# robjermy/CMVS-PMVS

Measured on AMD Instinct MI355X. Metric: refined patches/sec + NCC evals/sec, 50-view 4K synthetic, 1/2/4/8 GPU, higher is better.
Workload: dtype f32 (f64 optimizer)

## Files before the change

cmvs-pmvs_amd/csrc/pmvs_api.cpp:

```cpp
#include <hip/hip_runtime.h>

#include <algorithm>
#include <climits>
#include <cmath>
#include <cstdarg>
#include <cstdio>
#include <cstdlib>
#include <cstring>
#include <chrono>
#include <condition_variable>
#include <mutex>
#include <string>
#include <vector>

#include "../../include/pmvs_amd.h"
#include "pmvs_features.h"
#include "pmvs_fmt.h"
#include "pmvs_launch.h"

using namespace pmvsdev;

namespace {

thread_local std::string g_err = "";
// ... 763 lines not shown
  }
  pmvs_status st = check_candidates(sc, in, n);
  if (st) return st;
  HIPCHK(hipSetDevice(sc->device));
  if ((st = ensure(sc->cand, n)) || (st = ensure(sc->res, n))) return st;
  HIPCHK(hipMemcpyAsync(sc->cand.p, in, n * sizeof(pmvs_candidate), hipMemcpyHostToDevice, sc->stream));
  if ((st = pmvs_refine_batch_device(sc, sc->cand.p, n, sc->res.p))) return st;
  HIPCHK(hipMemcpyAsync(out, sc->res.p, n * sizeof(pmvs_refined), hipMemcpyDeviceToHost, sc->stream));
  return pmvs_scene_sync(sc, stats);
}

pmvs_status pmvs_selftest_math(int32_t device, int32_t op, const double* in, double* out, int32_t n) {
  if (!in || !out || n <= 0) return fail(PMVS_EINVAL, "null argument");
  HIPCHK(hipSetDevice(device));
  double *di = nullptr, *dout = nullptr;
  HIPCHK(hipMalloc((void**)&di, n * sizeof(double)));
  hipError_t e = hipMalloc((void**)&dout, n * sizeof(double));
  if (e == hipSuccess) e = hipMemcpy(di, in, n * sizeof(double), hipMemcpyHostToDevice);
  if (e == hipSuccess) e = launch_math_selftest(op, di, dout, n, nullptr);
  if (e == hipSuccess) e = hipMemcpy(out, dout, n * sizeof(double), hipMemcpyDeviceToHost);
  (void)hipFree(di);
  if (dout) (void)hipFree(dout);
  if (e != hipSuccess) return fail(PMVS_EDEVICE, "math selftest: %s", hipGetErrorString(e));
  return PMVS_OK;
}

pmvs_status pmvs_selftest_lls(int32_t device, const float* A, const float* b, const int32_t* offsets, int32_t nsys,
                              float* x) {
  if (!A || !b || !offsets || !x || nsys <= 0) return fail(PMVS_EINVAL, "null argument");
  for (int k = 0; k < nsys; ++k)
    if (offsets[k + 1] - offsets[k] < 5) return fail(PMVS_EINVAL, "system %d has fewer than 5 rows", k);
  HIPCHK(hipSetDevice(device));
  HIPCHK(lls_selftest(A, b, offsets, nsys, offsets[nsys], x));
  return PMVS_OK;
}

pmvs_status pmvs_selftest_bobyqa(int32_t device, int32_t mode, int32_t kind, const double* x0, int32_t n,
                                 int32_t maxeval, double* out, double* ms) {
  if (!x0 || !out || n <= 0) return fail(PMVS_EINVAL, "null argument");
  HIPCHK(hipSetDevice(device));
  double *dx = nullptr, *dout = nullptr;
  hipEvent_t e0 = nullptr, e1 = nullptr;
  HIPCHK(hipMalloc((void**)&dx, 3 * n * sizeof(double)));
  hipError_t e = hipMalloc((void**)&dout, 6 * n * sizeof(double));
  if (e == hipSuccess) e = hipEventCreate(&e0);
  if (e == hipSuccess) e = hipEventCreate(&e1);
  if (e == hipSuccess) e = hipMemcpy(dx, x0, 3 * n * sizeof(double), hipMemcpyHostToDevice);
  if (e == hipSuccess) e = hipEventRecord(e0, nullptr);
  if (e == hipSuccess) e = launch_bobyqa_selftest(mode, kind, dx, n, maxeval, dout, nullptr);
  if (e == hipSuccess) e = hipEventRecord(e1, nullptr);
  if (e == hipSuccess) e = hipMemcpy(out, dout, 6 * n * sizeof(double), hipMemcpyDeviceToHost);
  float t = 0;
  if (e == hipSuccess) e = hipEventElapsedTime(&t, e0, e1);
  if (ms) *ms = t;
  if (e0) (void)hipEventDestroy(e0);
  if (e1) (void)hipEventDestroy(e1);
  (void)hipFree(dx);
  if (dout) (void)hipFree(dout);
  if (e != hipSuccess) return fail(PMVS_EDEVICE, "bobyqa selftest: %s", hipGetErrorString(e));
  return PMVS_OK;
}

}

pmvs_status pmvs_patch_colors(pmvs_scene* sc, int32_t n, const float* coords4, const int32_t* nimg,
                              const int32_t* images_flat, int32_t* colors_out) {
// ... 957 lines not shown
```

cmvs-pmvs_amd/csrc/pmvs_filter.hip:

```cpp
#include <hip/hip_runtime.h>
#include <hipcub/hipcub.hpp>

#include <algorithm>
#include <chrono>
#include <cmath>
#include <cstdio>
#include <cstddef>
#include <cstdlib>
#include <cstring>
#include <functional>
#include <mutex>
#include <unordered_map>
#include <vector>

#include "pmvs_device.h"
#include "pmvs_launch.h"
#include "pmvs_layout.h"
#include "pmvs_queue.h"

namespace pmvsdev {

#ifndef PMVS_NB_CAP
#define PMVS_NB_CAP 1024
#endif
// ... 2647 lines not shown
  FCHK(memset_big(B.cellcnt, 0, (c.ncells + 1) * sizeof(int), c.st));
  if (e > 0) {
    hipLaunchKernelGGL(cell_hist_kernel, dim3(nblk(e)), dim3(256), 0, c.st, B.keys2, e, B.cellcnt);
    hipLaunchKernelGGL(items_kernel, dim3(nblk(e)), dim3(256), 0, c.st, B.keys2, e, items);
  }
  FCHK(cub_run(B.temp, [&](void* t, size_t& tb) {
    return hipcub::DeviceScan::ExclusiveSum(t, tb, B.cellcnt.p, csr_off, (int)(c.ncells + 1), c.st);
  }));
  return hipGetLastError();
}

__global__ void flag_order_kernel(const int* __restrict__ v, const int* __restrict__ order, int na, int* __restrict__ f) {
  const int i = blockIdx.x * blockDim.x + threadIdx.x;
  if (i < na) f[i] = v[order[i]] != 0;
}
__global__ void scatter_order_kernel(const int* __restrict__ f, const int* __restrict__ off, const int* __restrict__ order,
                                     int na, int* __restrict__ out) {
  const int i = blockIdx.x * blockDim.x + threadIdx.x;
  if (i < na && f[i]) out[off[i]] = order[i];
}

__global__ void pack_bits_kernel(const int* __restrict__ f, int n, unsigned* __restrict__ bits) {
  const int w = blockIdx.x * blockDim.x + threadIdx.x;
  if (w * 32 >= n) return;
  unsigned v = 0u;
  for (int b = 0; b < 32 && w * 32 + b < n; ++b) v |= (f[w * 32 + b] != 0 ? 1u : 0u) << b;
  bits[w] = v;
}
__global__ void unpack_bits_kernel(const unsigned* __restrict__ bits, int n, int* __restrict__ f) {
  const int k = blockIdx.x * blockDim.x + threadIdx.x;
  if (k < n) f[k] = (bits[k >> 5] >> (k & 31)) & 1u;
}

static int lab_jump() {
  static const int v = getenv("PMVS_LAB_JUMP") ? std::max(1, atoi(getenv("PMVS_LAB_JUMP"))) : 1;
  return v;
}
__global__ void lab_init_kernel(int* __restrict__ lab, int* __restrict__ active, int na) {
  const int i = blockIdx.x * blockDim.x + threadIdx.x;
  if (i < na) {
    lab[i] = i;
    active[i] = 1;
  }
}
__global__ void lab_relax_kernel(const int* __restrict__ eoff, const int* __restrict__ edges, int na, int* lab,
                                 int* active, int all, int* changed, int jump) {
  const int i = blockIdx.x * blockDim.x + threadIdx.x;
  if (i >= na) return;
  if (!all && !jump && active[i] == 0) return;
  const int l0 = lab[i], l1 = lab[l0];
  const bool jumped = l1 < l0 && atomicMin(&lab[i], l1) > l1;
  if (jumped) atomicOr(changed, 1);
  if (!all && !jumped && active[i] == 0) return;
  if (atomicExch(&active[i], 0) == 0 && !all && !jumped) return;
  const int li = atomicAdd(&lab[i], 0);
  bool any = false;
  for (int e = eoff[i]; e < eoff[i + 1]; ++e) {
    const int j = edges[e];
    if (li < lab[j] && atomicMin(&lab[j], li) > li) {
      atomicOr(&active[j], 1);
      any = true;
    }
  }
  if (any) atomicOr(changed, 1);
}
__global__ void lab_count_kernel(const int* __restrict__ lab, int na, int* __restrict__ csize) {
  const int i = blockIdx.x * blockDim.x + threadIdx.x;
  const int l = (i < na) ? lab[i] : -1;
  const int l0 = __shfl(l, 0, 64);
  const unsigned long long same = __ballot(i < na && l == l0);
  if (i < na && l != l0) atomicAdd(&csize[l], 1);
  if ((threadIdx.x & 63) == 0 && same) atomicAdd(&csize[l0], (int)__popcll(same));
}
__global__ void lab_flags_kernel(const int* __restrict__ lab, const int* __restrict__ csize, const int* __restrict__ order,
                                 int na, int threshold, int* __restrict__ flags) {
  const int i = blockIdx.x * blockDim.x + threadIdx.x;
  if (i < na && csize[lab[i]] < threshold) flags[order[i]] = 1;
}

static hipError_t collect(Ctx& c) {
  FilterBuffers& B = c.B;
  FCHK(hipMemsetAsync(B.counters, 0, 8 * sizeof(int), c.st));
  hipLaunchKernelGGL(first_cell_kernel, dim3(std::min(nblk((long long)c.n * kLG), 2048u)), dim3(256), 0, c.st, c.s, c.P, c.n,
                     B.preg, B.tgoff, B.keys,
                     B.counters);
  FCHK(cub_run(B.temp, [&](void* t, size_t& tb) {
    return hipcub::DeviceRadixSort::SortKeys(t, tb, B.keys.p, B.keys2.p, c.n, 32, 32 + cell_bits(c.ncells), c.st);
  }));
  FCHK(read_int(B.counters, &c.nalive, c.st));
  FCHK(hipMemsetAsync(B.rank, 0xff, c.n * sizeof(int), c.st));
  if (c.nalive > 0)
    hipLaunchKernelGGL(rank_kernel, dim3(nblk(c.nalive)), dim3(256), 0, c.st, B.keys2, c.nalive, B.order, B.rank);
  hipLaunchKernelGGL(hot_kernel, dim3(nblk(c.n)), dim3(256), 0, c.st, c.s, c.P, c.n, B.hot);
  return hipGetLastError();
}

static hipError_t set_dm_vgrids(Ctx& c, int additive) {
// ... 232 lines not shown
    }
    fprintf(stderr, "[filter] neighbours: max unique %d, overflowed %d of %d; first: %d %d %d\n", mx, ov, c.nalive,
            cnts[ord[0]], c.nalive > 1 ? cnts[ord[1]] : 0, c.nalive > 2 ? cnts[ord[2]] : 0);
  }
  FCHK(read_int(B.counters + 3, overflow, st));
  if (part) {
    long long ovf = 0;
    FCHK(merge_flags(*overflow, &ovf));
    *overflow = (int)ovf;
    if (inject && inj_where == 'g') return hipErrorOutOfMemory;
  }
  {
    int errs[2] = {0, 0};
    FCHK(hipMemcpy(errs, B.counters + 6, 2 * sizeof(int), hipMemcpyDeviceToHost));
    if (errs[0]) {
      fprintf(stderr, "[filter] neighbor kernel bounds violations: %d (first code %d)\n", errs[0], errs[1]);
      return hipErrorIllegalAddress;
    }
  }
  FCHK(apply_flags(c, &counts[2]));
  FCHK(set_dm_vgrids(c, 1));
  if (c.nalive) {
    const int na = c.nalive;
    hipLaunchKernelGGL(group_edges_kernel, dim3(nblk(na)), dim3(256), 0, st, s, c.dev(), 0, B.edge_off, B.cnt, B.edges);
    FCHK(hipMemsetAsync(B.cnt + na, 0, sizeof(int), st));
    FCHK(cub_run(B.temp, [&](void* t, size_t& tb) { return hipcub::DeviceScan::ExclusiveSum(t, tb, B.cnt.p, B.edge_off.p, na + 1, st); }));
    int ne = 0;
    FCHK(read_int(B.edge_off + na, &ne, st));
    if ((size_t)ne > B.edges.cap) FCHK(B.edges.alloc((size_t)ne * 2));
    hipLaunchKernelGGL(group_edges_kernel, dim3(nblk(na)), dim3(256), 0, st, s, c.dev(), 1, B.edge_off, B.cnt, B.edges);
    const int threshold = std::max(20, na / 10000);
    int* lab = B.need;
    int* csize = B.list;
    int* changed = B.counters + 5;
    int* active = B.list;
    hipLaunchKernelGGL(lab_init_kernel, dim3(nblk(na)), dim3(256), 0, st, lab, active, na);
    int sweep = 0;
    for (int it = 0;; ++it) {
      const bool verify = (it % 9) == 8;
      FCHK(hipMemsetAsync(changed, 0, sizeof(int), st));
      for (int r = 0; r < (verify ? 1 : 8); ++r) {
        if (ne)
          hipLaunchKernelGGL(lab_relax_kernel, dim3(nblk(na)), dim3(256), 0, st, B.edge_off, B.edges, na, lab, active,
                             verify ? 1 : 0, changed, (sweep++ % lab_jump()) == 0 ? 1 : 0);
      }
      int ch = 0;
      FCHK(read_int(changed, &ch, st));
      if (verify && !ch) break;
      if (!verify && !ch) it = 9 * (it / 9) + 7;
      if (it > 9 * (na + 1)) return hipErrorIllegalState;
    }
    FCHK(hipMemsetAsync(csize, 0, na * sizeof(int), st));
    hipLaunchKernelGGL(lab_count_kernel, dim3(nblk(na)), dim3(256), 0, st, lab, na, csize);
    FCHK(hipMemsetAsync(B.flags, 0, n * sizeof(int), st));
    hipLaunchKernelGGL(lab_flags_kernel, dim3(nblk(na)), dim3(256), 0, st, lab, csize, B.order, na, threshold, B.flags);
    hipLaunchKernelGGL(flag_rank_kernel, dim3(nblk(na)), dim3(256), 0, st, dP, B.order, na);
    hipLaunchKernelGGL(clear_fixed_kernel, dim3(nblk(n)), dim3(256), 0, st, dP, n, B.flags);
    FCHK(apply_flags(c, &counts[3]));
  }
  dbg(st, "groups");
  FCHK(set_dm_vgrids(c, 1));
  FCHK(build_lists(c, 0));
  FCHK(collect(c));
  hipLaunchKernelGGL(keep_kernel, dim3(nblk(n)), dim3(256), 0, st, n, B.preg, B.rank, keep_dev);
  int lovf = 0;
  FCHK(read_int(B.counters + 8, &lovf, st));
  if (lovf) return hipErrorNotSupported;
  return hipGetLastError();
}

static void nb_prof_dump(const char* what) {
#if defined(NB_PROFILE)
  unsigned long long h[3][8];
  if (hipDeviceSynchronize() != hipSuccess || hipMemcpyFromSymbol(h, HIP_SYMBOL(g_nb_prof), sizeof(h)) != hipSuccess) return;
  fprintf(stderr, "{\"nb_prof\": \"%s\"", what);
  for (int k = 0; k < 3; ++k) {
    fprintf(stderr, ", \"k%d\": [", k);
    for (int i = 0; i < 8; ++i) fprintf(stderr, "%s%llu", i ? ", " : "", h[k][i]);
    fprintf(stderr, "]");
  }
  fprintf(stderr, "}\n");
  std::memset(h, 0, sizeof(h));
  (void)hipMemcpyToSymbol(HIP_SYMBOL(g_nb_prof), h, sizeof(h));
#else
// ... 1064 lines not shown
__global__ __launch_bounds__(64) void lls_selftest_kernel(const float* __restrict__ A, const float* __restrict__ b,
                                                          const int* __restrict__ off, int nsys, double* __restrict__ scratch,
                                                          float* __restrict__ x) {
  __shared__ NbLds L;
  const int sys = blockIdx.x;
  if (sys >= nsys) return;
  const int o = off[sys], n = off[sys + 1] - off[sys];
  double* M = scratch + (size_t)o * 6;
  double* r = M + (size_t)n * 5;
  for (int i = threadIdx.x; i < n; i += 64) {
    for (int j = 0; j < 5; ++j) M[(size_t)i * 5 + j] = (double)A[(size_t)(o + i) * 5 + j];
    r[i] = (double)b[o + i];
  }
  __threadfence_block();
  __syncthreads();
  lls5_wave(L, M, r, n);
  if (threadIdx.x < 5) x[(size_t)sys * 5 + threadIdx.x] = L.x[threadIdx.x];
}

hipError_t lls_selftest(const float* A, const float* b, const int* off, int nsys, int total, float* x) {
  DevBuf<float> dA, db, dx;
  DevBuf<int> doff;
  DevBuf<double> scr;
  FCHK(dA.alloc((size_t)total * 5)); FCHK(db.alloc((size_t)total)); FCHK(dx.alloc((size_t)nsys * 5));
  FCHK(doff.alloc((size_t)nsys + 1)); FCHK(scr.alloc((size_t)total * 6));
  FCHK(hipMemcpy(dA, A, (size_t)total * 5 * sizeof(float), hipMemcpyHostToDevice));
  FCHK(hipMemcpy(db, b, (size_t)total * sizeof(float), hipMemcpyHostToDevice));
  FCHK(hipMemcpy(doff, off, (size_t)(nsys + 1) * sizeof(int), hipMemcpyHostToDevice));
  hipLaunchKernelGGL(lls_selftest_kernel, dim3(nsys), dim3(64), 0, nullptr, dA.p, db.p, doff.p, nsys, scr.p, dx.p);
  FCHK(hipGetLastError());
  return hipMemcpy(x, dx, (size_t)nsys * 5 * sizeof(float), hipMemcpyDeviceToHost);
}

__global__ __launch_bounds__(64) void compact_kernel(const pmvs_patch* __restrict__ src, int n, const int* __restrict__ keep,
                                                     const int* __restrict__ pos, pmvs_patch* __restrict__ dst) {
  const int k = blockIdx.x;
  if (k >= n || !keep[k]) return;
  const unsigned* a = reinterpret_cast<const unsigned*>(&src[k]);
  unsigned* b = reinterpret_cast<unsigned*>(&dst[pos[k]]);
  for (int w = threadIdx.x; w < (int)(sizeof(pmvs_patch) / 4); w += 64) b[w] = a[w];
}

__global__ void fill_int_kernel(int* __restrict__ a, int n, int v) {
  const int k = blockIdx.x * blockDim.x + threadIdx.x;
  if (k < n) a[k] = v;
}

hipError_t compact_model(FilterBuffers& B, const pmvs_patch* src, int n, const int* keep, const CompactDst& dst_for,
                         int* nkept, hipStream_t st) {
  *nkept = 0;
  if (n <= 0) return hipSuccess;
  FCHK(B.reserve(n, B.cap_cells, 0, B.cap_grid));
  FCHK(hipMemcpyAsync(B.cnt, keep, n * sizeof(int), hipMemcpyDeviceToDevice, st));
  FCHK(hipMemsetAsync(B.cnt + n, 0, sizeof(int), st));
  FCHK(cub_run(B.temp, [&](void* t, size_t& tb) { return hipcub::DeviceScan::ExclusiveSum(t, tb, B.cnt.p, B.off.p, n + 1, st); }));
  FCHK(read_int(B.off + n, nkept, st));
  pmvs_patch* dst = nullptr;
  FCHK(dst_for(*nkept, &dst));
  if (*nkept > 0) hipLaunchKernelGGL(compact_kernel, dim3(n), dim3(64), 0, st, src, n, keep, B.off, dst);
  return hipGetLastError();
}

hipError_t fill_int(int* a, int n, int v, hipStream_t st) {
  if (n > 0) hipLaunchKernelGGL(fill_int_kernel, dim3(nblk(n)), dim3(256), 0, st, a, n, v);
  return hipGetLastError();
}
// ... 149 lines not shown
```

cmvs-pmvs_amd/csrc/pmvs_launch.h:

```cpp
#pragma once
#include <hip/hip_runtime.h>
#include "pmvs_device.h"
#include "pmvs_devbuf.h"
#include "pmvs_refine_layouts.h"
#include <functional>
#include <memory>
#include <utility>
#include <vector>

namespace pmvsdev {

inline hipError_t memset_big(void* p, int value, size_t bytes, hipStream_t st) {
  constexpr size_t kPiece = size_t(1) << 30;
  char* c = static_cast<char*>(p);
  for (size_t off = 0; off < bytes; off += kPiece) {
    const hipError_t e = hipMemsetAsync(c + off, value, bytes - off < kPiece ? bytes - off : kPiece, st);
    if (e != hipSuccess) return e;
  }
  return hipSuccess;
}
struct PinnedBuf {
  void* p = nullptr;
  size_t cap = 0;
  PinnedBuf() = default;
// ... 70 lines not shown
hipError_t export_order(const DScene& s, const pmvs_patch* P, int n, int max_gwidth, int* sorted, int* cnt_i, int* cnt_v,
                        hipStream_t st);

struct TextArrays {
  const float* fields = nullptr;
  const int* colors = nullptr;
  const long long *image_off = nullptr, *vimage_off = nullptr;
  const int *image_ids = nullptr, *vimage_ids = nullptr;
};
hipError_t text_offsets(int kind, const TextArrays& in, int n, long long header_bytes, long long* d_off, hipStream_t st);
hipError_t text_write(int kind, const TextArrays& in, int n, const long long* d_off, char* d_out, hipStream_t st);
hipError_t launch_format_selftest(int precision, const float* d_in, int n, char* d_out, int* d_len, hipStream_t st);

struct DepthMapArrays {
  int* patch = nullptr;
  float *depth = nullptr, *normal = nullptr, *ncc = nullptr;
};
hipError_t depth_map_pass(const DScene& s, const pmvs_patch* P, int n, const int* src, const long long* d_off,
                          long long cells, const DepthMapArrays& out, hipStream_t st);

struct alignas(64) PHot {
  float coord[4];
  float normal[4];
  float dscale, ncc, unit0, pad[5];
};
struct FilterBuffers {
  PinnedBuf pin;
  DevBuf<Reg> preg, vreg, safe;
  DevBuf<unsigned long long> keys, keys2, dpkey;
  DevBuf<long long> tgoff;
  DevBuf<int> cnt, off, cellcnt, pg_off, pg_items, vp_off, vp_items, order, rank, flags, need, list, counters, edge_off,
      edges;
  DevBuf<PHot> hot;
  DevBuf<double> scratch;
  DevBuf<char> temp;
  DevBuf<unsigned> rbits;
  DevBuf<float4> coordc;
  DevBuf<unsigned long long> vrows, used;
  DevBuf<float4> normalc;
  DevBuf<int> refpos;
  DevBuf<char> xr;
  DevBuf<float> qf;
  DevBuf<double> qrows;
  DevBuf<int4> qjobs;
  DevBuf<unsigned long long> qctr;
  DevBuf<unsigned long long> qkeys, qkeys2;
  DevBuf<int> qcrows, qoff;
  size_t cap_qrows = 0;
  DevBuf<int> ovf_items;
  DevBuf<double> scratch_big;
  int cap_n = 0, cap_grid = 0;
  long long cap_cells = 0;
  size_t cap_e = 0;
  hipError_t reserve(int n, long long ncells, int tnum, int grid);
  hipError_t ensure_entries(size_t e, int vis);
  void release() { *this = FilterBuffers(); }
};

hipError_t launch_filter_refimage(const DScene& s, pmvs_patch* P, const int* list, int m, int grid, hipStream_t stream,
                                  int* refpos = nullptr, int rank = 0, int world = 1);
hipError_t launch_apply_refpos(const DScene& s, pmvs_patch* P, const int* list, int m, const int* allpos, int world,
                               hipStream_t stream);

constexpr int kMaxWave = 65536;
struct CommitWork;
struct CommitWorkDelete {
// ... 54 lines not shown
  ExchangeDevFn exchange_dev;
};
hipError_t filter_pass(const DScene& s, FilterBuffers& B, pmvs_patch* dP, int n, long long ncells, const long long* h_tgoff,
                       int grid, hipStream_t st, int counts[4], int* overflow, int* keep_dev, const Shard* sh = nullptr,
                       bool* handled = nullptr);
hipError_t expand_pass(const DScene& s, FilterBuffers& B, ExpandBuffers& X, pmvs_patch*& dP, size_t& dP_cap, int n0,
                       const int* d_alive, int cap, long long ncells, const long long* h_tgoff, int wave, int cthr,
                       int flags, int grid, hipStream_t st, const RefineFn& refine, const Shard& sh, long long stats[8],
                       int* n_out, int min_cands = 0);
using CompactDst = std::function<hipError_t(int, pmvs_patch**)>;
hipError_t compact_model(FilterBuffers& B, const pmvs_patch* src, int n, const int* keep, const CompactDst& dst_for,
                         int* nkept, hipStream_t st);
hipError_t fill_int(int* a, int n, int v, hipStream_t st);
void d2h_stage_release(hipStream_t st);

struct ClusterMaps {
  const unsigned char* shared_t;
  const int* ids;
  const int* id2idx;
  int maxid;
};
struct ClusterBuffers {
  DevBuf<BRec> send, recv;
  DevBuf<pmvs_patch> ins;
  DevBuf<int> flags, pos, cnts;
  DevBuf<char> temp;
};
hipError_t drop_foreign(FilterBuffers& B, const pmvs_patch* src, int n, const CompactDst& dst_for, int* n_out,
                        hipStream_t st);
hipError_t cluster_exchange(const DScene& s, ClusterBuffers& CB, const ClusterMaps& cm, const pmvs_patch* src, int n,
                            pmvs_patch*& dst, size_t& dst_cap, int* n_out, const Shard& sh, hipStream_t st,
                            long long xstats[3], bool& agreed);
hipError_t lls_selftest(const float* A, const float* b, const int* off, int nsys, int total, float* x);

struct SeedInput {
  const pmvs_point* points;
  const int* npts;
  const int* vis_off;
  const int* vis;
  int sequence;
  float angle0;
  std::vector<const uint8_t*> mask_level;
  int batch, per_cell;
  int lookahead;
  int spec_near;
};
struct SeedOutput {
  std::vector<pmvs_patch> seeds;
  long long stats[8];
  double gen_ms = 0, refine_ms = 0, wall_ms = 0;
};
hipError_t seed_pass(const DScene& s, const std::vector<DView>& hv, const SeedInput& in, hipStream_t st,
                     const RefineFn& refine, SeedOutput& out);
}
```

cmvs-pmvs_amd/pmvs_amd.py:

```python
from __future__ import annotations

import ctypes as C
import os
from dataclasses import dataclass, field
from typing import List, Optional, Sequence

import numpy as np

HERE = os.path.dirname(os.path.abspath(__file__))
LIB_PATH = os.environ.get("PMVS_AMD_LIB", os.path.join(HERE, "libpmvs_amd.so"))

MAX_IMAGES = 128
MAX_TAU = 16

ACCEPTED, FAIL_PRE, FAIL_POST, FAIL_OVERFLOW = 0, 1, 2, 3
FIX_FOREIGN = 2

CANDIDATE_DTYPE = np.dtype(
    [("coord", "<f4", 4), ("normal", "<f4", 4), ("dscale", "<f4"), ("num_images", "<i4"),
     ("images", "<i4", MAX_IMAGES)], align=True)
REFINED_DTYPE = np.dtype(
    [("status", "<i4"), ("refine_code", "<i4"), ("evals", "<i4"), ("num_images", "<i4"),
     ("coord", "<f4", 4), ("normal", "<f4", 4), ("ncc", "<f4"), ("dscale", "<f4"), ("ascale", "<f4"),
     ("tmp", "<f4"), ("timages", "<i4"), ("reserved", "<i4"), ("images", "<i4", MAX_IMAGES),
# ... 103 lines not shown
               [(k, C.c_float) for k in ("threshold", "set_edge", "max_angle", "quad")] + \
               [(k, C.c_int32) for k in ("num_timages", "num_oimages", "num_bindexes")] + \
               [(k, C.POINTER(C.c_int32)) for k in ("timages", "oimages", "bindexes", "visdata2_offsets",
                                                      "visdata2")]


class SynthParams(C.Structure):
    _fields_ = [("num_views", C.c_int32), ("num_targets", C.c_int32), ("width", C.c_int32),
                ("height", C.c_int32), ("supersample", C.c_int32), ("level", C.c_int32),
                ("seed", C.c_uint64), ("ring_radius", C.c_double), ("height_offset", C.c_double),
                ("focal_scale", C.c_double), ("arc_step_deg", C.c_double), ("gain_sigma", C.c_double),
                ("bias_sigma", C.c_double), ("noise_sigma", C.c_double), ("lowtex", C.c_double),
                ("occluder_radius", C.c_double), ("render_first", C.c_int32), ("render_count", C.c_int32)]


HARD = dict(gain_sigma=0.15, bias_sigma=0.04, noise_sigma=0.08, lowtex=0.5, occluder_radius=0.3)


EXPORTS = ["pmvs_last_error", "pmvs_device_count", "pmvs_scene_create", "pmvs_scene_destroy",
           "pmvs_set_thresholds", "pmvs_scene_get_level", "pmvs_grab_tex", "pmvs_incc_eval",
           "pmvs_refine_batch", "pmvs_refine_batch_device", "pmvs_scene_sync", "pmvs_synth_ring",
           "pmvs_synth_candidates", "pmvs_selftest_math", "pmvs_selftest_bobyqa", "pmvs_camera_load",
           "pmvs_ppm_load", "pmvs_options_load", "pmvs_options_free", "pmvs_write_patches", "pmvs_write_pset",
           "pmvs_write_ply", "pmvs_patch_colors", "pmvs_filter_run",
           "pmvs_expand_run", "pmvs_expand_fetch", "pmvs_run_loop", "pmvs_loop_fetch", "pmvs_loop_hash",
           "pmvs_loop_export_sizes", "pmvs_loop_export", "pmvs_export_patches_sizes", "pmvs_export_patches",
           "pmvs_depth_map_layout", "pmvs_loop_depth_maps", "pmvs_depth_maps_patches", "pmvs_write_pfm",
           "pmvs_loop_text", "pmvs_text_patches", "pmvs_selftest_format",
           "pmvs_scene_set_shard", "pmvs_scene_set_shard_rccl", "pmvs_scene_set_cluster",
           "pmvs_scene_set_cluster_rccl", "pmvs_rccl_unique_id",
           "pmvs_rccl_create", "pmvs_rccl_destroy", "pmvs_rccl_allgather", "pmvs_rccl_allgather_device",
           "pmvs_tcp_create", "pmvs_tcp_allgather", "pmvs_tcp_destroy", "pmvs_thread_exchange_create",
           "pmvs_thread_exchange_ctx", "pmvs_thread_allgather", "pmvs_thread_exchange_destroy", "pmvs_detect_features",
           "pmvs_seed_run", "pmvs_seed_fetch", "pmvs_selftest_lls", "pmvs_image_load", "pmvs_pnm_mask_load", "pmvs_set_edge"]

ALLGATHER_FN = C.CFUNCTYPE(C.c_int, C.c_void_p, C.c_void_p, C.c_int64, C.c_void_p)

_lib = None


def load_library(path: str = LIB_PATH) -> C.CDLL:
    global _lib
    if _lib is not None:
        return _lib
    if not os.path.exists(path):
        raise RuntimeError(f"{path} not built: run `make -C cmvs-pmvs_amd` (no CPU fallback exists)")
    lib = C.CDLL(path)
    lib.pmvs_last_error.restype = C.c_char_p
    lib.pmvs_device_count.restype = C.c_int32
    lib.pmvs_scene_create.argtypes = [C.POINTER(SceneDesc), C.c_int32, C.POINTER(C.c_void_p)]
    lib.pmvs_scene_destroy.argtypes = [C.c_void_p]
    lib.pmvs_scene_destroy.restype = None
    lib.pmvs_set_thresholds.argtypes = [C.c_void_p, C.c_float, C.c_float, C.c_int32]
    lib.pmvs_scene_get_level.argtypes = [C.c_void_p, C.c_int32, C.c_int32, C.c_void_p,
                                         C.POINTER(C.c_int32), C.POINTER(C.c_int32)]
    lib.pmvs_grab_tex.argtypes = [C.c_void_p, C.c_void_p, C.c_int32, C.c_void_p, C.c_void_p]
    lib.pmvs_detect_features.argtypes = [C.c_void_p, C.c_int32, C.c_int32, C.c_void_p, C.c_int32,
                                         C.POINTER(C.c_int32)]
    lib.pmvs_seed_run.argtypes = [C.c_void_p, C.c_void_p, C.c_void_p, C.c_int32, C.c_void_p, C.c_int32,
                                  C.POINTER(C.c_int32), C.POINTER(SeedStats)]
    lib.pmvs_seed_fetch.argtypes = [C.c_void_p, C.c_void_p, C.c_int32]
    lib.pmvs_incc_eval.argtypes = [C.c_void_p, C.c_void_p, C.c_int32, C.c_void_p, C.POINTER(Stats)]
    lib.pmvs_refine_batch.argtypes = [C.c_void_p, C.c_void_p, C.c_int32, C.c_void_p, C.POINTER(Stats)]
    lib.pmvs_refine_batch_device.argtypes = [C.c_void_p, C.c_void_p, C.c_int32, C.c_void_p]
    lib.pmvs_scene_sync.argtypes = [C.c_void_p, C.POINTER(Stats)]
    lib.pmvs_synth_ring.argtypes = [C.POINTER(SynthParams), C.c_void_p, C.c_void_p, C.c_int32]
    lib.pmvs_synth_candidates.argtypes = [C.POINTER(SynthParams), C.c_void_p, C.c_int32, C.c_uint64,
                                          C.c_float, C.c_float, C.c_void_p]
    lib.pmvs_selftest_bobyqa.argtypes = [C.c_int32, C.c_int32, C.c_int32, C.c_void_p, C.c_int32, C.c_int32,
                                         C.c_void_p, C.POINTER(C.c_double)]
    lib.pmvs_selftest_lls.argtypes = [C.c_int32, C.c_void_p, C.c_void_p, C.c_void_p, C.c_int32, C.c_void_p]
    lib.pmvs_selftest_math.argtypes = [C.c_int32, C.c_int32, C.c_void_p, C.c_void_p, C.c_int32]
    lib.pmvs_camera_load.argtypes = [C.c_char_p, C.c_void_p]
    lib.pmvs_image_load.argtypes = [C.c_char_p, C.POINTER(C.c_int32), C.POINTER(C.c_int32), C.c_void_p]
    lib.pmvs_pnm_mask_load.argtypes = [C.c_char_p, C.POINTER(C.c_int32), C.POINTER(C.c_int32), C.c_void_p]
    lib.pmvs_set_edge.argtypes = [C.c_void_p, C.c_int32, C.c_int32, C.c_float, C.c_void_p]
    lib.pmvs_ppm_load.argtypes = [C.c_char_p, C.POINTER(C.c_int32), C.POINTER(C.c_int32), C.c_void_p]
    lib.pmvs_options_load.argtypes = [C.c_char_p, C.c_char_p, C.POINTER(C.POINTER(Options))]
    lib.pmvs_options_free.argtypes = [C.POINTER(Options)]
    lib.pmvs_options_free.restype = None
    lib.pmvs_write_patches.argtypes = [C.c_char_p, C.c_int32] + [C.c_void_p] * 5
    lib.pmvs_write_pset.argtypes = [C.c_char_p, C.c_int32, C.c_void_p]
    lib.pmvs_write_ply.argtypes = [C.c_char_p, C.c_int32, C.c_void_p, C.c_void_p]
    lib.pmvs_patch_colors.argtypes = [C.c_void_p, C.c_int32] + [C.c_void_p] * 4
    lib.pmvs_filter_run.argtypes = [C.c_void_p, C.c_void_p, C.c_int32, C.c_void_p, C.POINTER(FilterStats)]
    lib.pmvs_expand_run.argtypes = [C.c_void_p, C.c_void_p, C.c_void_p, C.c_int32, C.c_int32, C.c_int32, C.c_int32, C.c_int32,
                                    C.c_void_p, C.c_void_p, C.c_int32, C.POINTER(C.c_int32), C.POINTER(ExpandStats)]
    lib.pmvs_expand_fetch.argtypes = [C.c_void_p, C.c_void_p, C.c_void_p, C.c_int32]
    lib.pmvs_run_loop.argtypes = [C.c_void_p, C.c_void_p, C.c_int32, C.c_float, C.c_int32, C.c_int32, C.c_int32, C.c_int32,
                                  C.c_int32, C.POINTER(C.c_int32), C.c_void_p]
    lib.pmvs_loop_fetch.argtypes = [C.c_void_p, C.c_void_p, C.c_int32]
    lib.pmvs_loop_hash.argtypes = [C.c_void_p, C.POINTER(C.c_uint64)]
    lib.pmvs_loop_export_sizes.argtypes = [C.c_void_p, C.POINTER(ExportSizes)]
    lib.pmvs_loop_export.argtypes = [C.c_void_p, C.c_int32, C.c_void_p, C.POINTER(ExportBuffers)]
    lib.pmvs_export_patches_sizes.argtypes = [C.c_void_p, C.c_void_p, C.c_int32, C.POINTER(ExportSizes)]
    lib.pmvs_export_patches.argtypes = [C.c_void_p, C.c_void_p, C.c_int32, C.c_int32, C.c_void_p,
                                        C.POINTER(ExportBuffers)]
    lib.pmvs_depth_map_layout.argtypes = [C.c_void_p, C.c_void_p, C.c_void_p]
    lib.pmvs_loop_depth_maps.argtypes = [C.c_void_p, C.c_int32, C.POINTER(DepthMapBuffers)]
    lib.pmvs_depth_maps_patches.argtypes = [C.c_void_p, C.c_void_p, C.c_int32, C.c_int32, C.POINTER(DepthMapBuffers)]
    lib.pmvs_write_pfm.argtypes = [C.c_char_p, C.c_int32, C.c_int32, C.c_void_p]
    lib.pmvs_loop_text.argtypes = [C.c_void_p, C.c_int32, C.c_int32, C.c_void_p, C.c_void_p, C.c_int64,
                                   C.POINTER(C.c_int64)]
    lib.pmvs_text_patches.argtypes = [C.c_void_p, C.c_void_p, C.c_int32, C.c_int32, C.c_int32, C.c_void_p, C.c_void_p,
# ... 434 lines not shown
        parts.append(r)
    npts = np.array([len(p) for p in parts], np.int32)
    flat = np.concatenate(parts) if parts and npts.sum() else np.zeros(1, POINT_DTYPE)
    return np.ascontiguousarray(flat), npts


def selftest_math(op: int, x: np.ndarray, device: int = 0) -> np.ndarray:
    x = np.ascontiguousarray(x, np.float64)
    out = np.zeros_like(x)
    _check(load_library().pmvs_selftest_math(device, op, _ptr(x), _ptr(out), len(x)))
    return out


def selftest_format(precision: int, x: np.ndarray, device: int = 0):
    x = np.ascontiguousarray(x, np.float32).reshape(-1)
    out = np.zeros((len(x), 24), np.uint8)
    ln = np.zeros(len(x), np.int32)
    if len(x):
        _check(load_library().pmvs_selftest_format(device, precision, _ptr(x), len(x), _ptr(out), _ptr(ln)))
    raw = out.tobytes()
    return [raw[24 * i:24 * i + int(k)] for i, k in enumerate(ln)]


def selftest_lls(systems, device: int = 0) -> np.ndarray:
    A = np.ascontiguousarray(np.concatenate([np.asarray(a, np.float32).reshape(-1, 5) for a, _ in systems]))
    b = np.ascontiguousarray(np.concatenate([np.asarray(v, np.float32).reshape(-1) for _, v in systems]))
    off = np.zeros(len(systems) + 1, np.int32)
    off[1:] = np.cumsum([len(v) for _, v in systems])
    x = np.zeros((len(systems), 5), np.float32)
    _check(load_library().pmvs_selftest_lls(device, _ptr(A), _ptr(b), _ptr(off), len(systems), _ptr(x)))
    return x


def selftest_bobyqa(kind: int, x0: np.ndarray, mode: int = 0, maxeval: int = 1000, device: int = 0):
    x0 = np.ascontiguousarray(x0, np.float64).reshape(-1, 3)
    out = np.zeros((len(x0), 6), np.float64)
    ms = C.c_double()
    _check(load_library().pmvs_selftest_bobyqa(device, mode, kind, _ptr(x0), len(x0), maxeval, _ptr(out), C.byref(ms)))
    return out, ms.value


def camera_load(path: str) -> np.ndarray:
    out = np.zeros(12, np.float32)
    _check(load_library().pmvs_camera_load(path.encode(), _ptr(out)))
    return out.reshape(3, 4)


def ppm_load(path: str) -> np.ndarray:
    lib = load_library()
    w, h = C.c_int32(), C.c_int32()
    _check(lib.pmvs_ppm_load(path.encode(), C.byref(w), C.byref(h), None))
    img = np.zeros((h.value, w.value, 3), np.uint8)
    _check(lib.pmvs_ppm_load(path.encode(), C.byref(w), C.byref(h), _ptr(img)))
    return img


def image_load(path: str) -> np.ndarray:
    lib = load_library()
    w, h = C.c_int32(), C.c_int32()
    _check(lib.pmvs_image_load(path.encode(), C.byref(w), C.byref(h), None))
    img = np.zeros((h.value, w.value, 3), np.uint8)
    _check(lib.pmvs_image_load(path.encode(), C.byref(w), C.byref(h), _ptr(img)))
    return img


def mask_load(path: str) -> np.ndarray:
# ... 227 lines not shown
```

include/pmvs_amd.h:

```cpp
#ifndef PMVS_AMD_H
#define PMVS_AMD_H

#include <stdint.h>

#ifdef __cplusplus
extern "C" {
#endif

#define PMVS_MAX_IMAGES 128
#define PMVS_MAX_TARGETS 256
#define PMVS_MAX_TAU 16
#define PMVS_MAX_LEVEL 4
#define PMVS_MAX_NEIGHBOURS 16384

typedef enum pmvs_status {
  PMVS_OK = 0,
  PMVS_EINVAL = 1,
  PMVS_EDEVICE = 2,
  PMVS_ENOMEM = 3,
  PMVS_EUNSUPPORTED = 4
} pmvs_status;

typedef enum pmvs_candidate_status {
  PMVS_ACCEPTED = 0,
// ... 101 lines not shown

pmvs_status pmvs_set_thresholds(pmvs_scene* scene, float ncc, float ncc_before, int32_t depth);

pmvs_status pmvs_scene_get_level(pmvs_scene* scene, int32_t view, int32_t level, uint8_t* out,
                                 int32_t* width, int32_t* height);

typedef struct pmvs_point {
  float x, y, response;
  int32_t type;
} pmvs_point;

pmvs_status pmvs_detect_features(pmvs_scene* scene, int32_t view, int32_t fcsize, pmvs_point* out, int32_t cap,
                                 int32_t* n_out);

pmvs_status pmvs_grab_tex(pmvs_scene* scene, const pmvs_tex_query* q, int32_t n, float* out_tex,
                          int32_t* out_valid);

pmvs_status pmvs_incc_eval(pmvs_scene* scene, const pmvs_eval_query* q, int32_t n, double* out_f,
                           pmvs_stats* stats);

pmvs_status pmvs_refine_batch(pmvs_scene* scene, const pmvs_candidate* in, int32_t n,
                              pmvs_refined* out, pmvs_stats* stats);

pmvs_status pmvs_refine_batch_device(pmvs_scene* scene, const pmvs_candidate* d_in, int32_t n,
                                     pmvs_refined* d_out);
pmvs_status pmvs_scene_sync(pmvs_scene* scene, pmvs_stats* stats);


pmvs_status pmvs_selftest_math(int32_t device, int32_t op, const double* in, double* out, int32_t n);

pmvs_status pmvs_selftest_lls(int32_t device, const float* A, const float* b, const int32_t* offsets, int32_t nsys,
                              float* x);

pmvs_status pmvs_selftest_bobyqa(int32_t device, int32_t mode, int32_t kind, const double* x0, int32_t n,
                                 int32_t maxeval, double* out, double* ms);

typedef struct pmvs_patch {
  float coord[4], normal[4];
  float ncc, dscale, ascale, tmp;
  int32_t timages, flag, fix, num_images, num_vimages, dflag;
  int16_t images[PMVS_MAX_IMAGES];
  int16_t grids[PMVS_MAX_IMAGES][2];
  int16_t vimages[PMVS_MAX_IMAGES];
  int16_t vgrids[PMVS_MAX_IMAGES][2];
} pmvs_patch;

#define PMVS_FIX_FOREIGN 2

typedef struct pmvs_filter_stats {
  int64_t input, removed_outside, removed_exact, removed_neighbor, removed_groups, kept;
  double kernel_ms;
} pmvs_filter_stats;

pmvs_status pmvs_filter_run(pmvs_scene* scene, pmvs_patch* patches, int32_t n, int32_t* keep,
                            pmvs_filter_stats* stats);

#define PMVS_EXPAND_AFTER_SEEDS 1
#define PMVS_EXPAND_MAX_WAVES(n) ((int32_t)((uint32_t)(n) << 8))
typedef struct pmvs_expand_stats {
  int64_t parents, candidates, fail_prep, fail_pre, fail_post, fail_commit, added, waves;
  double wall_ms;
  int64_t refined, evals, tex_valid;
  double refine_ms;
  int64_t refine_launches;
  int64_t tex_valid_small;
  double refine_ms_small;
// ... 160 lines not shown
```

Before: 963,300.

## Use frontier worklist label propagation for filter group component labeling

Replaces the fixed full-sweep label propagation in the patch-group filter with a hybrid fixpoint. It runs full relax sweeps while many vertices are active, and switches to a compacted frontier list processed by 16-lane groups once the active set is small. Host readbacks happen only once per batch of sweeps. This cuts wasted full-grid sweeps and host syncs on long-tail convergence, at the cost of more control logic, atomics on list counters, and a workspace buffer. It also adds a labels selftest API and optional tracing.

```diff
diff --git a/cmvs-pmvs_amd/csrc/pmvs_api.cpp b/cmvs-pmvs_amd/csrc/pmvs_api.cpp
--- a/cmvs-pmvs_amd/csrc/pmvs_api.cpp
+++ b/cmvs-pmvs_amd/csrc/pmvs_api.cpp
@@ -819,6 +819,17 @@
     if (offsets[k + 1] - offsets[k] < 5) return fail(PMVS_EINVAL, "system %d has fewer than 5 rows", k);
   HIPCHK(hipSetDevice(device));
   HIPCHK(lls_selftest(A, b, offsets, nsys, offsets[nsys], x));
+  return PMVS_OK;
+}
+
+pmvs_status pmvs_labels_selftest(const int32_t* eoff, const int32_t* edges, int32_t n, int32_t* lab_out) {
+  if (!eoff || !lab_out || n <= 0 || eoff[0] != 0) return fail(PMVS_EINVAL, "null argument or empty graph");
+  for (int i = 0; i < n; ++i)
+    if (eoff[i + 1] < eoff[i]) return fail(PMVS_EINVAL, "edge offsets decrease at vertex %d", i);
+  if (eoff[n] > 0 && !edges) return fail(PMVS_EINVAL, "null argument");
+  for (int e = 0; e < eoff[n]; ++e)
+    if (edges[e] < 0 || edges[e] >= n) return fail(PMVS_EINVAL, "edge %d leaves the graph", e);
+  HIPCHK(labels_selftest(eoff, edges, n, lab_out));
   return PMVS_OK;
 }
 
diff --git a/cmvs-pmvs_amd/csrc/pmvs_filter.hip b/cmvs-pmvs_amd/csrc/pmvs_filter.hip
--- a/cmvs-pmvs_amd/csrc/pmvs_filter.hip
+++ b/cmvs-pmvs_amd/csrc/pmvs_filter.hip
@@ -2703,10 +2703,6 @@
   if (k < n) f[k] = (bits[k >> 5] >> (k & 31)) & 1u;
 }
 
-static int lab_jump() {
-  static const int v = getenv("PMVS_LAB_JUMP") ? std::max(1, atoi(getenv("PMVS_LAB_JUMP"))) : 1;
-  return v;
-}
 __global__ void lab_init_kernel(int* __restrict__ lab, int* __restrict__ active, int na) {
   const int i = blockIdx.x * blockDim.x + threadIdx.x;
   if (i < na) {
@@ -2715,15 +2711,18 @@
   }
 }
 __global__ void lab_relax_kernel(const int* __restrict__ eoff, const int* __restrict__ edges, int na, int* lab,
-                                 int* active, int all, int* changed, int jump) {
+                                 int* active, int all, int* changed, int* nact) {
   const int i = blockIdx.x * blockDim.x + threadIdx.x;
   if (i >= na) return;
-  if (!all && !jump && active[i] == 0) return;
   const int l0 = lab[i], l1 = lab[l0];
   const bool jumped = l1 < l0 && atomicMin(&lab[i], l1) > l1;
   if (jumped) atomicOr(changed, 1);
   if (!all && !jumped && active[i] == 0) return;
   if (atomicExch(&active[i], 0) == 0 && !all && !jumped) return;
+  if (nact) {
+    const unsigned long long m = __ballot(1);
+    if ((int)(threadIdx.x & 63) == __ffsll((long long)m) - 1) atomicAdd(nact, (int)__popcll(m));
+  }
   const int li = atomicAdd(&lab[i], 0);
   bool any = false;
   for (int e = eoff[i]; e < eoff[i + 1]; ++e) {
@@ -2734,6 +2733,119 @@
     }
   }
   if (any) atomicOr(changed, 1);
+}
+constexpr int kLabLanes = 16;
+__global__ void lab_list_kernel(const int* __restrict__ eoff, const int* __restrict__ edges, int na, int* lab, int* active,
+                                int* lists, int* ctl, int k, int* nact) {
+  const int n = min(ctl[1 + k % 3], na);
+  const int* cur = lists + (size_t)(k & 1) * na;
+  int* nxt = lists + (size_t)((k + 1) & 1) * na;
+  int* nnxt = ctl + 1 + (k + 1) % 3;
+  if (blockIdx.x == 0 && threadIdx.x == 0) {
+    ctl[1 + (k + 2) % 3] = 0;
+    if (nact) *nact = n;
+  }
+  const int g = threadIdx.x & (kLabLanes - 1);
+  const int ngroups = gridDim.x * (blockDim.x / kLabLanes);
+  for (int t = (blockIdx.x * blockDim.x + threadIdx.x) / kLabLanes; t < n; t += ngroups) {
+    const int i = cur[t];
+    const int e0 = eoff[i], e1 = eoff[i + 1];
+    int li = -1;
+    if (g == 0 && atomicExch(&active[i], 0) != 0) {
+      const int l0 = atomicAdd(&lab[i], 0), l1 = lab[l0];
+      li = l0;
+      if (l1 < l0) {
+        atomicMin(&lab[i], l1);
+        li = l1;
+      }
+    }
+    li = __shfl(li, 0, kLabLanes);
+    if (li < 0) continue;
+    for (int e = e0 + g; e < e1; e += kLabLanes) {
+      const int j = edges[e];
+      if (li < lab[j] && atomicMin(&lab[j], li) > li && atomicOr(&active[j], 1) == 0) {
+        const int p = atomicAdd(nnxt, 1);
+        if (p < na) nxt[p] = j;
+      }
+    }
+  }
+}
+__global__ void lab_collect_kernel(const int* __restrict__ active, int na, int* __restrict__ list, int* ctl) {
+  const int i = blockIdx.x * blockDim.x + threadIdx.x;
+  const bool f = i < na && active[i] != 0;
+  const unsigned long long m = __ballot(f);
+  if (!m) return;
+  const int lane = threadIdx.x & 63, lead = __ffsll((long long)m) - 1;
+  int base = 0;
+  if (lane == lead) base = atomicAdd(&ctl[1], (int)__popcll(m));
+  base = __shfl(base, lead, 64);
+  if (f) list[base + (int)__popcll(m & ((1ull << lane) - 1ull))] = i;
+}
+
+constexpr int kLabFullBatch = 8;
+constexpr int kLabListShare = 16;
+constexpr int kLabTraceMax = 1 << 16;
+static hipError_t label_fixpoint(const int* eoff, const int* edges, int na, int ne, int* lab, int* active,
+                                 DevBuf<int>& work, hipStream_t st) {
+  const char* e_max = getenv("PMVS_LAB_LIST_MAX");
+  const char* e_batch = getenv("PMVS_LAB_BATCH");
+  const bool trace = getenv("PMVS_LAB_TRACE") != nullptr;
+  const long long list_max = e_max ? std::max(0ll, atoll(e_max)) : na / kLabListShare;
+  const int batch = e_batch ? std::max(1, atoi(e_batch)) : 32;
+  const bool jump_all = getenv("PMVS_LAB_JUMP") ? atoi(getenv("PMVS_LAB_JUMP")) != 0 : true;
+  FCHK(work.grow(8 + 2 * (size_t)na + (trace ? kLabTraceMax : 0)));
+  int* ctl = work;
+  int* lists = work + 8;
+  int* tr = trace ? work + 8 + 2 * (size_t)na : nullptr;
+  if (trace) {
+    FCHK(hipMemsetAsync(tr, 0, kLabTraceMax * sizeof(int), st));
+    FCHK(hipStreamSynchronize(st));
+  }
+  const auto t0 = std::chrono::steady_clock::now();
+  hipLaunchKernelGGL(lab_init_kernel, dim3(nblk(na)), dim3(256), 0, st, lab, active, na);
+  if (ne == 0) return hipGetLastError();
+  const unsigned lgrid = std::min(nblk((long long)na * kLabLanes), 2048u);
+  enum { kFull, kList, kVerify } mode = kFull;
+  std::string forms;
+  int sweeps = 0, reads = 0, k = 0;
+  auto slot = [&]() { return (trace && sweeps < kLabTraceMax) ? tr + sweeps : nullptr; };
+  for (long long it = 0;; ++it) {
+    if (mode == kList)
+      for (int r = 0; r < batch; ++r, ++k, ++sweeps) {
+        hipLaunchKernelGGL(lab_list_kernel, dim3(lgrid), dim3(256), 0, st, eoff, edges, na, lab, active, lists, ctl, k,
+                           slot());
+        if (trace) forms += 'L';
+      }
+    if (mode != kList || jump_all) {
+      FCHK(hipMemsetAsync(ctl, 0, 4 * sizeof(int), st));
+      const int nfull = mode == kFull ? std::min(batch, kLabFullBatch) : 1;
+      for (int r = 0; r < nfull; ++r, ++sweeps) {
+        hipLaunchKernelGGL(lab_relax_kernel, dim3(nblk(na)), dim3(256), 0, st, eoff, edges, na, lab, active,
+                           mode == kVerify ? 1 : 0, ctl, slot());
+        if (trace) forms += mode == kVerify ? 'V' : 'F';
+      }
+      hipLaunchKernelGGL(lab_collect_kernel, dim3(nblk(na)), dim3(256), 0, st, active, na, lists, ctl);
+      k = 0;
+    }
+    int h[4] = {0, 0, 0, 0};
+    FCHK(d2h_sync(st, {{h, ctl, sizeof(h)}}));
+    ++reads;
+    if (mode == kVerify && !h[0]) break;
+    const int next = h[1 + k % 3];
+    mode = next == 0 ? kVerify : next <= list_max ? kList : kFull;
+    if (it > 9ll * (na + 1)) return hipErrorIllegalState;
+  }
+  if (trace) {
+    const int nt = std::min(sweeps, kLabTraceMax);
+    std::vector<int> h((size_t)nt);
+    FCHK(hipMemcpy(h.data(), tr, (size_t)nt * sizeof(int), hipMemcpyDeviceToHost));
+    const double ms = std::chrono::duration<double, std::milli>(std::chrono::steady_clock::now() - t0).count();
+    fprintf(stderr, "[labels] na=%d ne=%d list_max=%lld batch=%d sweeps=%d reads=%d ms=%.3f:", na, ne, list_max, batch, sweeps,
+            reads, ms);
+    for (int i = 0; i < nt; ++i) fprintf(stderr, " %c%d", forms[(size_t)i], h[(size_t)i]);
+    fprintf(stderr, "\n");
+  }
+  return hipGetLastError();
 }
 __global__ void lab_count_kernel(const int* __restrict__ lab, int na, int* __restrict__ csize) {
   const int i = blockIdx.x * blockDim.x + threadIdx.x;
@@ -3032,24 +3144,8 @@
     const int threshold = std::max(20, na / 10000);
     int* lab = B.need;
     int* csize = B.list;
-    int* changed = B.counters + 5;
     int* active = B.list;
-    hipLaunchKernelGGL(lab_init_kernel, dim3(nblk(na)), dim3(256), 0, st, lab, active, na);
-    int sweep = 0;
-    for (int it = 0;; ++it) {
-      const bool verify = (it % 9) == 8;
-      FCHK(hipMemsetAsync(changed, 0, sizeof(int), st));
-      for (int r = 0; r < (verify ? 1 : 8); ++r) {
-        if (ne)
-          hipLaunchKernelGGL(lab_relax_kernel, dim3(nblk(na)), dim3(256), 0, st, B.edge_off, B.edges, na, lab, active,
-                             verify ? 1 : 0, changed, (sweep++ % lab_jump()) == 0 ? 1 : 0);
-      }
-      int ch = 0;
-      FCHK(read_int(changed, &ch, st));
-      if (verify && !ch) break;
-      if (!verify && !ch) it = 9 * (it / 9) + 7;
-      if (it > 9 * (na + 1)) return hipErrorIllegalState;
-    }
+    FCHK(label_fixpoint(B.edge_off, B.edges, na, ne, lab, active, B.lab_work, st));
     FCHK(hipMemsetAsync(csize, 0, na * sizeof(int), st));
     hipLaunchKernelGGL(lab_count_kernel, dim3(nblk(na)), dim3(256), 0, st, lab, na, csize);
     FCHK(hipMemsetAsync(B.flags, 0, n * sizeof(int), st));
@@ -4180,6 +4276,22 @@
   return hipMemcpy(x, dx, (size_t)nsys * 5 * sizeof(float), hipMemcpyDeviceToHost);
 }
 
+hipError_t labels_selftest(const int* eoff, const int* edges, int n, int* lab) {
+  const int ne = eoff[n];
+  DevBuf<int> doff, dedges, dlab, dactive, work;
+  FCHK(doff.alloc((size_t)n + 1)); FCHK(dedges.alloc((size_t)ne)); FCHK(dlab.alloc((size_t)n)); FCHK(dactive.alloc((size_t)n));
+  FCHK(hipMemcpy(doff, eoff, ((size_t)n + 1) * sizeof(int), hipMemcpyHostToDevice));
+  if (ne) FCHK(hipMemcpy(dedges, edges, (size_t)ne * sizeof(int), hipMemcpyHostToDevice));
+  hipStream_t st = nullptr;
+  FCHK(hipStreamCreateWithFlags(&st, hipStreamNonBlocking));
+  hipError_t e = label_fixpoint(doff, dedges, n, ne, dlab, dactive, work, st);
+  if (e == hipSuccess) e = hipStreamSynchronize(st);
+  d2h_stage_release(st);
+  (void)hipStreamDestroy(st);
+  FCHK(e);
+  return hipMemcpy(lab, dlab, (size_t)n * sizeof(int), hipMemcpyDeviceToHost);
+}
+
 __global__ __launch_bounds__(64) void compact_kernel(const pmvs_patch* __restrict__ src, int n, const int* __restrict__ keep,
                                                      const int* __restrict__ pos, pmvs_patch* __restrict__ dst) {
   const int k = blockIdx.x;
diff --git a/cmvs-pmvs_amd/csrc/pmvs_launch.h b/cmvs-pmvs_amd/csrc/pmvs_launch.h
--- a/cmvs-pmvs_amd/csrc/pmvs_launch.h
+++ b/cmvs-pmvs_amd/csrc/pmvs_launch.h
@@ -126,6 +126,7 @@
   DevBuf<int> cnt, off, cellcnt, pg_off, pg_items, vp_off, vp_items, order, rank, flags, need, list, counters, edge_off,
       edges;
   DevBuf<PHot> hot;
+  DevBuf<int> lab_work;
   DevBuf<double> scratch;
   DevBuf<char> temp;
   DevBuf<unsigned> rbits;
@@ -246,6 +247,7 @@
                             pmvs_patch*& dst, size_t& dst_cap, int* n_out, const Shard& sh, hipStream_t st,
                             long long xstats[3], bool& agreed);
 hipError_t lls_selftest(const float* A, const float* b, const int* off, int nsys, int total, float* x);
+hipError_t labels_selftest(const int* eoff, const int* edges, int n, int* lab);
 
 struct SeedInput {
   const pmvs_point* points;
diff --git a/cmvs-pmvs_amd/pmvs_amd.py b/cmvs-pmvs_amd/pmvs_amd.py
--- a/cmvs-pmvs_amd/pmvs_amd.py
+++ b/cmvs-pmvs_amd/pmvs_amd.py
@@ -159,7 +159,7 @@
            "pmvs_rccl_create", "pmvs_rccl_destroy", "pmvs_rccl_allgather", "pmvs_rccl_allgather_device",
            "pmvs_tcp_create", "pmvs_tcp_allgather", "pmvs_tcp_destroy", "pmvs_thread_exchange_create",
            "pmvs_thread_exchange_ctx", "pmvs_thread_allgather", "pmvs_thread_exchange_destroy", "pmvs_detect_features",
-           "pmvs_seed_run", "pmvs_seed_fetch", "pmvs_selftest_lls", "pmvs_image_load", "pmvs_pnm_mask_load", "pmvs_set_edge"]
+           "pmvs_seed_run", "pmvs_seed_fetch", "pmvs_selftest_lls", "pmvs_labels_selftest", "pmvs_image_load", "pmvs_pnm_mask_load", "pmvs_set_edge"]
 
 ALLGATHER_FN = C.CFUNCTYPE(C.c_int, C.c_void_p, C.c_void_p, C.c_int64, C.c_void_p)
 
@@ -197,6 +197,7 @@
     lib.pmvs_selftest_bobyqa.argtypes = [C.c_int32, C.c_int32, C.c_int32, C.c_void_p, C.c_int32, C.c_int32,
                                          C.c_void_p, C.POINTER(C.c_double)]
     lib.pmvs_selftest_lls.argtypes = [C.c_int32, C.c_void_p, C.c_void_p, C.c_void_p, C.c_int32, C.c_void_p]
+    lib.pmvs_labels_selftest.argtypes = [C.c_void_p, C.c_void_p, C.c_int32, C.c_void_p]
     lib.pmvs_selftest_math.argtypes = [C.c_int32, C.c_int32, C.c_void_p, C.c_void_p, C.c_int32]
     lib.pmvs_camera_load.argtypes = [C.c_char_p, C.c_void_p]
     lib.pmvs_image_load.argtypes = [C.c_char_p, C.POINTER(C.c_int32), C.POINTER(C.c_int32), C.c_void_p]
@@ -697,6 +698,16 @@
     return x
 
 
+def labels_selftest(eoff, edges) -> np.ndarray:
+    eoff = np.ascontiguousarray(eoff, np.int32)
+    edges = np.ascontiguousarray(edges, np.int32)
+    if len(edges) == 0:
+        edges = np.zeros(1, np.int32)
+    lab = np.full(len(eoff) - 1, -1, np.int32)
+    _check(load_library().pmvs_labels_selftest(_ptr(eoff), _ptr(edges), len(eoff) - 1, _ptr(lab)))
+    return lab
+
+
 def selftest_bobyqa(kind: int, x0: np.ndarray, mode: int = 0, maxeval: int = 1000, device: int = 0):
     x0 = np.ascontiguousarray(x0, np.float64).reshape(-1, 3)
     out = np.zeros((len(x0), 6), np.float64)
diff --git a/include/pmvs_amd.h b/include/pmvs_amd.h
--- a/include/pmvs_amd.h
+++ b/include/pmvs_amd.h
@@ -157,6 +157,8 @@
 pmvs_status pmvs_selftest_lls(int32_t device, const float* A, const float* b, const int32_t* offsets, int32_t nsys,
                               float* x);
 
+pmvs_status pmvs_labels_selftest(const int32_t* eoff, const int32_t* edges, int32_t n, int32_t* lab_out);
+
 pmvs_status pmvs_selftest_bobyqa(int32_t device, int32_t mode, int32_t kind, const double* x0, int32_t n,
                                  int32_t maxeval, double* out, double* ms);
 
```

New measurement: 962,200. About the same (-0.1%).
